# Youngju-Na/UFORecon

Measured on AMD Instinct MI355X. Metric: rays/s (per-ray volume-rendering path, 64+64 hierarchical samples, DTU-shaped 3-view 512x640), higher is better.
Workload: dtype f32; 1 GPU; configs[1]: full 512x640 frame = 327680 rays, 3 source views, 64+64 samples, rays sharded by row tiles over 1 GPU(s), depth/RGB tiles all-gathered; rays_per_frame=327680, chunk_rays=4096, side_streams=3

## Files before the change

### uforecon_amd/csrc/api_ray.hip

```cpp
#include "api_common.h"

using namespace ufr;
using namespace ufr::api;

namespace {
__global__ void order_pe_kernel(float* __restrict__ table, int SN) {
  int i = blockIdx.x * blockDim.x + threadIdx.x;
  if (i >= SN * 8) return;
  int pos = i >> 3, jj = i & 7;
  double ang = (double)pos / pow(10000.0, 2.0 * (double)(jj / 2) / 8.0);
  table[i] = (float)((jj & 1) ? cos(ang) : sin(ang));
}
}

namespace ufr {
hipError_t launch_order_pe(float* table, int SN, hipStream_t s) {
  hipLaunchKernelGGL(order_pe_kernel, dim3((SN * 8 + 255) / 256), dim3(256), 0, s, table, SN);
  return hipGetLastError();
}
}

namespace {
struct AggregateWs { float *token0, *order_pe; };
AggregateWs carve_aggregate(Carver& c, int RN, int SN) {
  AggregateWs w;
  w.token0 = c.f32((size_t)RN * SN * UFR_TOKEN_DIM);
  w.order_pe = c.f32((size_t)SN * 8);
  return w;
}

int aggregate_impl(const void* packed, const float* x_tokens, const float* x_point, const float* rgb, const float* dir, int RN, int SN,
                   int NV, float* radiance, float* srdf, float* token0, float* order_pe, bool pe_ready,
                   float* view_out, float* ray_out, bool lowp, int* status, hipStream_t s) {
  UFR_REQUIRE((unsigned long long)RN * SN * (NV + 1) * UFR_TOKEN_DIM < (1ull << 30),
              "view transformer: %d x %d points x %d tokens exceed the 2^30 token values one call addresses; chunk the points", RN, SN, NV + 1);
  UFR_TIMED("view_transformer", s, launch_view_transformer(static_cast<const float*>(packed), x_tokens, x_point, rgb, dir, RN * SN, NV,
      token0, radiance, view_out, lowp, status, s));
  if (!pe_ready) UFR_HIP(launch_order_pe(order_pe, SN, s));
  UFR_TIMED("ray_transformer", s, launch_ray_transformer(static_cast<const float*>(packed), token0, nullptr, order_pe, RN, SN, srdf,
      ray_out, lowp, status, s));
  return UFR_OK;
}
}

extern "C" {

int ufr_sample_fixed(const float* near, const float* far, const float* U, float* z_out, int32_t RN, int32_t SN,
                     ufr_stream stream) {
  UFR_REQUIRE(near && far && U && z_out, "ufr_sample_fixed: null argument");
  UFR_REQUIRE(RN > 0 && SN >= 2, "ufr_sample_fixed: RN=%d SN=%d", RN, SN);
  UFR_HIP(launch_sample_fixed(near, far, U, RN, z_out, RN, SN, static_cast<hipStream_t>(stream)));
  return UFR_OK;
// ... 23 lines not shown
  return UFR_OK;
}

int ufr_project_gather(const ufr_frame* frame, const ufr_raw_weights* raw, const float* ray_o, int32_t ray_o_stride,
                       const float* ray_d, const float* z, int32_t RN, int32_t SN, float* x_tokens, float* rgb,
                       float* dir, float* sim8, float* vol24, float* xy, float* mask_z, const float* vol24_in,
                       const float* sim8_in, ufr_stream stream) {
  const FrameDev* f = frame_of(frame);
  UFR_REQUIRE(f, "ufr_project_gather: frame handle not prepared");
  UFR_REQUIRE(raw && ray_o && ray_d && z && x_tokens && rgb && dir, "ufr_project_gather: null argument");
  UFR_REQUIRE(ray_o_stride == 0 || ray_o_stride == 3, "ufr_project_gather: ray_o_stride must be 0 or 3");
  UFR_REQUIRE(RN > 0 && SN > 0, "ufr_project_gather: RN=%d SN=%d", RN, SN);
  UFR_REQUIRE(f->match || sim8_in, "ufr_project_gather: the frame has no matching features: sim8_in is required");
  UFR_REQUIRE(f->vol[0] || vol24_in, "ufr_project_gather: the frame has no volumes: vol24_in is required");
  UFR_TIMED("gather", static_cast<hipStream_t>(stream), launch_gather(*f, presim_of(raw), ray_o, ray_o_stride, ray_d, z, RN, SN, x_tokens,
      nullptr, rgb, dir, sim8, vol24, xy, mask_z, vol24_in, sim8_in, static_cast<hipStream_t>(stream)));
  return UFR_OK;
}

size_t ufr_aggregate_workspace_bytes(int32_t RN, int32_t SN, int32_t ) {
  return carved_bytes(carve_aggregate, RN, SN);
}

int ufr_aggregate(const void* packed_weights, const float* x_tokens, const float* rgb, const float* dir, int32_t RN,
                  int32_t SN, int32_t NV, float* radiance, float* srdf, void* workspace, float* view_out,
                  float* ray_out, int32_t precision, ufr_stream stream) {
  UFR_REQUIRE(packed_weights && x_tokens && rgb && dir && radiance && srdf && workspace, "ufr_aggregate: null argument");
  UFR_CHECK(check_views("ufr_aggregate", NV));
  UFR_CHECK(check_ray_samples("ufr_aggregate", RN, SN));
  UFR_PRECISION(precision, lowp, "ufr_aggregate");
  hipStream_t s = static_cast<hipStream_t>(stream);
  UFR_STATUS_ENTER(sl, s, "ufr_aggregate");
  Carver c(workspace);
  const AggregateWs w = carve_aggregate(c, RN, SN);
  UFR_CHECK(aggregate_impl(packed_weights, x_tokens, nullptr, rgb, dir, RN, SN, NV, radiance, srdf, w.token0, w.order_pe, false,
                           view_out, ray_out, lowp, status_word(sl), s));
  return status_leave(sl, s);
}

int ufr_composite(const float* z, const float* radiance, const int32_t* row, const float* srdf, const float* variance,
                  int32_t RN, int32_t SN, float* rgb, float* depth, float* opacity, float* weight, ufr_stream stream) {
  UFR_REQUIRE(z && radiance && srdf && variance && depth, "ufr_composite: null argument");
  UFR_REQUIRE(RN > 0 && SN >= 2 && SN <= 256, "ufr_composite: SN=%d out of range [2,256]", SN);
  UFR_TIMED("composite", static_cast<hipStream_t>(stream), launch_composite(z, radiance, row, srdf, variance, RN, SN, rgb, depth, opacity,
      weight, nullptr, nullptr, static_cast<hipStream_t>(stream)));
  return UFR_OK;
}

int ufr_view_transform(const void* packed_weights, const float* x_tokens, const float* rgb, const float* dir, int32_t P,
                       int32_t NV, float* token0, float* radiance, int32_t precision, ufr_stream stream) {
  UFR_REQUIRE(packed_weights && x_tokens && rgb && dir && token0 && radiance, "ufr_view_transform: null argument");
  UFR_CHECK(check_views("ufr_view_transform", NV));
  UFR_REQUIRE(P > 0, "ufr_view_transform: P=%d", P);
  UFR_PRECISION(precision, lowp, "ufr_view_transform");
  hipStream_t s = static_cast<hipStream_t>(stream);
  UFR_STATUS_ENTER(sl, s, "ufr_view_transform");
  UFR_REQUIRE((unsigned long long)P * (NV + 1) * UFR_TOKEN_DIM < (1ull << 30),
              "ufr_view_transform: %d points x %d tokens exceed the 2^30 token values one call addresses; chunk the points", P, NV + 1);
  UFR_TIMED("view_transformer", s, launch_view_transformer(static_cast<const float*>(packed_weights), x_tokens, nullptr, rgb, dir, P, NV,
      token0, radiance, nullptr, lowp, status_word(sl), s));
  return status_leave(sl, s);
}

size_t ufr_ray_transform_workspace_bytes(int32_t SN) { return align_up((size_t)(SN > 0 ? SN : 1) * 8 * sizeof(float)); }

int ufr_ray_transform(const void* packed_weights, const float* token0, const int32_t* row, int32_t RN, int32_t SN,
                      float* srdf, void* workspace, int32_t precision, ufr_stream stream) {
  UFR_REQUIRE(packed_weights && token0 && srdf && workspace, "ufr_ray_transform: null argument");
  UFR_CHECK(check_ray_samples("ufr_ray_transform", RN, SN));
  UFR_PRECISION(precision, lowp, "ufr_ray_transform");
  hipStream_t s = static_cast<hipStream_t>(stream);
  UFR_STATUS_ENTER(sl, s, "ufr_ray_transform");
  float* order_pe = static_cast<float*>(workspace);
  UFR_HIP(launch_order_pe(order_pe, SN, s));
  UFR_TIMED("ray_transformer", s, launch_ray_transformer(static_cast<const float*>(packed_weights), token0, row, order_pe, RN, SN, srdf,
      nullptr, lowp, status_word(sl), s));
  return status_leave(sl, s);
}

int32_t ufr_default_chunk_rays(void) { return 4096; }

}

namespace {
struct RenderWs {
  float *ray_o, *rd, *near, *far, *camz, *z1, *w1, *srdf1, *depth1, *rgb1, *z2, *srdf2, *rad, *x, *xp, *rgbm, *dir, *token0,
      *pe1, *pe2, *z_new;
  int* row;
  size_t bytes;
};
RenderWs carve_render(void* ws, int R, int SN, int PN, int NV) {
  const size_t S2 = (size_t)SN + PN, Smax = S2 > (size_t)SN ? S2 : SN, Sg = (size_t)(SN > PN ? SN : PN);
  Carver c(ws);
  RenderWs r;
  r.ray_o = c.f32(4);
  r.rd = c.f32((size_t)R * 3);
  r.near = c.f32(R);
  r.far = c.f32(R);
  r.camz = c.f32(R);
  r.z1 = c.f32((size_t)R * SN);
  r.w1 = c.f32((size_t)R * SN);
  r.srdf1 = c.f32((size_t)R * SN);
  r.depth1 = c.f32(R);
  r.rgb1 = c.f32((size_t)R * 3);
  r.z2 = c.f32((size_t)R * S2);
  r.srdf2 = c.f32((size_t)R * S2);
  r.rad = c.f32((size_t)R * Smax * 3);
  r.x = c.f32((size_t)R * Sg * NV * kViewCols);
  r.xp = c.f32((size_t)R * Sg * kPointCols);
  r.rgbm = c.f32((size_t)R * Sg * NV * 4);
  r.dir = c.f32((size_t)R * Sg * NV * 4);
  r.z_new = c.f32((size_t)R * (PN > 0 ? PN : 1));
  r.row = c.take<int>((size_t)R * S2);
  r.token0 = c.f32((size_t)R * Smax * UFR_TOKEN_DIM);
  r.pe1 = c.f32((size_t)SN * 8);
  r.pe2 = c.f32(S2 * 8);
  r.bytes = c.off;
  return r;
}

constexpr int kMaxLanes = 4;
struct SidePool {
  hipStream_t s[kMaxLanes] = {};
  hipEvent_t fork = nullptr, join[kMaxLanes] = {};
  int n = 0;
};
// ... 19 lines not shown
                 int* status, hipStream_t s) {
  const int RN = a->RN, SN = a->SN, PN = a->coarse_only ? 0 : a->PN, NV = f->NV;
  const PreSim ps = presim_of(a->raw);
  const int S2 = SN + PN, HW = f->H * f->W;
  {
    ProfScope p("sampler", s);
    UFR_HIP(launch_ray_setup(a->ray_idx + r0, a->ray_d, a->cam_ray_d, HW, a->near_z, a->far_z, R, w.rd, w.near, w.far,
                             w.camz, a->ray_o, w.ray_o, s));
    UFR_HIP(launch_sample_fixed(w.near, w.far, a->U1 + r0, RN, w.z1, R, SN, s));
    if (!pe_ready) {
      UFR_HIP(launch_order_pe(w.pe1, SN, s));
      if (!a->coarse_only) UFR_HIP(launch_order_pe(w.pe2, S2, s));
      pe_ready = true;
    }
  }
  UFR_TIMED("gather", s, launch_gather(*f, ps, w.ray_o, 0, w.rd, w.z1, R, SN, w.x, w.xp, w.rgbm, w.dir, nullptr, nullptr, nullptr,
      nullptr, nullptr, nullptr, s));
  UFR_CHECK(aggregate_impl(a->packed_weights, w.x, w.xp, w.rgbm, w.dir, R, SN, NV, w.rad, w.srdf1, w.token0, w.pe1, true,
                           nullptr, nullptr, lowp, status, s));
  const bool last = a->coarse_only != 0;
  UFR_TIMED("composite", s, launch_composite(w.z1, w.rad, nullptr, w.srdf1, a->raw->variance, R, SN,
      last ? a->rgb + 3 * (size_t)r0 : w.rgb1, last ? a->depth + r0 : w.depth1, nullptr, w.w1, w.camz,
      (last && a->depth_z) ? a->depth_z + r0 : nullptr, s));
  if (last) {
    if (a->srdf) UFR_HIP(hipMemcpyAsync(a->srdf + (size_t)r0 * SN, w.srdf1, (size_t)R * SN * 4, hipMemcpyDeviceToDevice, s));
    if (a->z_all) UFR_HIP(hipMemcpyAsync(a->z_all + (size_t)r0 * SN, w.z1, (size_t)R * SN * 4, hipMemcpyDeviceToDevice, s));
    return UFR_OK;
  }
  UFR_TIMED("sampler", s, launch_importance_merge(w.w1, w.z1, a->U2 + r0, RN, nullptr, w.z2, R, SN, PN, w.z_new, w.row, s));
  UFR_TIMED("gather", s, launch_gather(*f, ps, w.ray_o, 0, w.rd, w.z_new, R, PN, w.x, w.xp, w.rgbm, w.dir, nullptr, nullptr, nullptr,
      nullptr, nullptr, nullptr, s));
  UFR_TIMED("view_transformer", s, launch_view_transformer(static_cast<const float*>(a->packed_weights), w.x, w.xp, w.rgbm, w.dir, R * PN,
      NV, w.token0 + (size_t)R * SN * UFR_TOKEN_DIM, w.rad + (size_t)R * SN * 3, nullptr, lowp, status, s));
  UFR_TIMED("ray_transformer", s, launch_ray_transformer(static_cast<const float*>(a->packed_weights), w.token0, w.row, w.pe2, R, S2,
      w.srdf2, nullptr, lowp, status, s));
  UFR_TIMED("composite", s, launch_composite(w.z2, w.rad, w.row, w.srdf2, a->raw->variance, R, S2, a->rgb + 3 * (size_t)r0, a->depth + r0,
      nullptr, nullptr, w.camz, a->depth_z ? a->depth_z + r0 : nullptr, s));
  if (a->srdf) UFR_HIP(hipMemcpyAsync(a->srdf + (size_t)r0 * S2, w.srdf2, (size_t)R * S2 * 4, hipMemcpyDeviceToDevice, s));
  if (a->z_all) UFR_HIP(hipMemcpyAsync(a->z_all + (size_t)r0 * S2, w.z2, (size_t)R * S2 * 4, hipMemcpyDeviceToDevice, s));
  return UFR_OK;
}
}

extern "C" {

size_t ufr_render_workspace_bytes(int32_t chunk_rays, int32_t SN, int32_t PN, int32_t NV) {
  if (chunk_rays <= 0) chunk_rays = ufr_default_chunk_rays();
// ... 69 lines not shown
```

### uforecon_amd/csrc/gather.hip

```cpp
#include <algorithm>
#include <cstdlib>
#include "ufr_device.h"
#include "ufr_internal.h"
#include "volume_sample.h"

namespace ufr {

__device__ __forceinline__ f32x4 lerp_tap4_buf(__amdgpu_buffer_rsrc_t r, unsigned base, int stride_bytes, const Tap2& t, unsigned c4) {
  f32x4 v[4];
#pragma unroll
  for (int k = 0; k < 4; ++k)
    v[k] = buf_ld4(r, t.o[k] >= 0 ? base + __umul24((unsigned)t.o[k], (unsigned)stride_bytes) + c4 : kBufOut);
  f32x4 acc;
#pragma unroll
  for (int e = 0; e < 4; ++e) {
    float a = mul_rn(v[0][e], t.w[0]);
    a = fmaf(v[1][e], t.w[1], a);
    a = fmaf(v[2][e], t.w[2], a);
    acc[e] = fmaf(v[3][e], t.w[3], a);
  }
  return acc;
}

typedef int i32x4 __attribute__((ext_vector_type(4)));
// ... 88 lines not shown
#define UFR_G_PHASE(i)                                                                 \
  {                                                                                    \
    const unsigned long long t_now = __builtin_readcyclecounter();                     \
    g_acc[i] = t_now - g_prev;                                                         \
    g_prev = t_now;                                                                    \
  }
#else
#define UFR_G_PHASE(i)
#endif

template <int NVT>
__global__ void __launch_bounds__(64 * NVT, kGatherMinW) gather_kernel(FrameDev f, PreSim ps, const float* __restrict__ ray_o,
                                                      int o_stride, const float* __restrict__ ray_d,
                                                      const float* __restrict__ zval, int P, int SN, int SG,
                                                      float* __restrict__ x_tokens, float* __restrict__ x_point,
                                                      float* __restrict__ rgb_out,
                                                      float* __restrict__ dir_out, float* __restrict__ sim8_out,
                                                      float* __restrict__ vol24_out, float* __restrict__ xy_out,
                                                      float* __restrict__ maskz_out,
                                                      const float* __restrict__ vol24_in,
                                                      const float* __restrict__ sim8_in) {
  extern __shared__ __attribute__((aligned(16))) float smem[];
  constexpr int NV = NVT;
  constexpr int npair = NV * (NV - 1) / 2;
  float* sh_sim = smem;
  float* sh_tapF = sh_sim + 64 * npair * 8;
  float* sh_tapM = sh_tapF + NV * 64 * 8;
  float* sh_vol = sh_tapF;
  constexpr int sim_slot = npair * 8;
  constexpr bool out_in_sim = sim_slot >= 48;
  float* sh_out = out_in_sim ? sh_sim + 8 : sh_tapF;
// ... 1 lines not shown
#ifdef UFR_PHASE_TIMING
  unsigned long long g_acc[8] = {};
  unsigned long long g_prev = __builtin_readcyclecounter();
#endif

  const int v = threadIdx.x >> 6, p = threadIdx.x & 63;
  const int vu = __builtin_amdgcn_readfirstlane(v);
  const int nb8 = (int)(gridDim.x / 8) * 8;
  const int blk = (int)blockIdx.x < nb8 ? (int)(blockIdx.x % 8) * (nb8 / 8) + (int)(blockIdx.x / 8) : (int)blockIdx.x;
  int pbase = blk * 64;
  if (SG) {
    const int rg = blk / SG;
    pbase = (kBlkRays * rg) * SN + kBlkSamples * (blk - rg * SG);
  }
  const auto point_of = [=](int lp) { return SG ? pbase + (int)((unsigned)lp % kBlkRays) * SN + (int)((unsigned)lp / kBlkRays) : pbase + lp; };
  const int pidx = point_of(p);
  const bool active = pidx < P;
  const int pc = active ? pidx : P - 1;
  const int ray = pc / SN;

  const float zz = zval[pc];
  const float* o = ray_o + (size_t)ray * o_stride;
  const float px = mul_add_unfused(zz, ray_d[3 * ray + 0], o[0]);
  const float py = mul_add_unfused(zz, ray_d[3 * ray + 1], o[1]);
  const float pz = mul_add_unfused(zz, ray_d[3 * ray + 2], o[2]);

  const float* M = f.pose[v];
  float qx = fmaf(M[2], pz, fmaf(M[1], py, mul_rn(M[0], px))) + M[3];
  float qy = fmaf(M[6], pz, fmaf(M[5], py, mul_rn(M[4], px))) + M[7];
  float qz = fmaf(M[10], pz, fmaf(M[9], py, mul_rn(M[8], px))) + M[11];
  const float mask_z = qz > 0.f ? 1.f : 0.f;
  const float x = qx / qz, y = qy / qz;
  if (active && xy_out) {
    xy_out[((size_t)v * P + pidx) * 2 + 0] = x;
    xy_out[((size_t)v * P + pidx) * 2 + 1] = y;
  }
  if (active && maskz_out) maskz_out[(size_t)v * P + pidx] = mask_z;

  const int row_cols = x_point ? kViewCols : UFR_TOKEN_DIM, pe_col = x_point ? 32 : 72;
  float* xrow = x_tokens + ((size_t)pc * NV + v) * row_cols;

  {
    put_tap(sh_tapF + (v * 64 + p) * 8, taps_zeros(unnorm2d_nac(x, f.w), unnorm2d_nac(y, f.h), f.w, f.h));
    put_tap(sh_tapM + (v * 64 + p) * 8, taps_border(unnorm2d_ac(x, f.w), unnorm2d_ac(y, f.h), f.w, f.h));
    Tap2 tf = taps_zeros(unnorm2d_nac(x, f.W), unnorm2d_nac(y, f.H), f.W, f.H);
    const unsigned img_px = (unsigned)(f.H * f.W);
    f32x4 c4 = lerp_tap4_buf(buf_rsrc(f.rgb + (size_t)vu * img_px * 4, img_px * 16u), 0u, 16, tf, 0u);
    const float inb = (x <= 1.f && x >= -1.f && y <= 1.f && y >= -1.f) ? 1.f : 0.f;
    c4[3] = inb * mask_z;
    if (active) st4(rgb_out + ((size_t)pidx * NV + v) * 4, c4);
    float dv[4];
    const __amdgpu_buffer_rsrc_t rdepth = buf_rsrc(f.depth + (size_t)vu * img_px, img_px * 4u);
#pragma unroll
    for (int k = 0; k < 4; ++k) dv[k] = buf_ld1(rdepth, tf.o[k] >= 0 ? (unsigned)tf.o[k] * 4u : kBufOut);
    const float dm = fmaf(dv[3], tf.w[3], fmaf(dv[2], tf.w[2], fmaf(dv[1], tf.w[1], mul_rn(dv[0], tf.w[0]))));
    const float* R = f.w2c_z[v];
    float zc = fmaf(R[2], pz, fmaf(R[1], py, mul_rn(R[0], px))) + R[3];
    float delta = dm - zc;
    float pe[8];
#pragma unroll
    for (int k = 0; k < 4; ++k) {
      const float fr = 3.14159274101257324f * (float)(1 << k);
      pe[2 * k] = sinf(mul_rn(delta, fr));
      pe[2 * k + 1] = sinf(fmaf(delta, fr, 1.57079637050628662f));
    }
    if (active) {
      st4(xrow + pe_col, f32x4{pe[0], pe[1], pe[2], pe[3]});
      st4(xrow + pe_col + 4, f32x4{pe[4], pe[5], pe[6], pe[7]});
    }
    float ax = px - f.ref_pos[0], ay = py - f.ref_pos[1], az = pz - f.ref_pos[2];
    float bx = px - f.cam_pos[v][0], by = py - f.cam_pos[v][1], bz = pz - f.cam_pos[v][2];
    const float ra = __builtin_amdgcn_rcpf(sqrtf(ax * ax + ay * ay + az * az));
    const float rb = __builtin_amdgcn_rcpf(sqrtf(bx * bx + by * by + bz * bz));
    if (active) st4(dir_out + ((size_t)pidx * NV + v) * 4, f32x4{ax * ra - bx * rb, ay * ra - by * rb, az * ra - bz * rb, 0.f});
  }

  __syncthreads();
  UFR_G_PHASE(0)

  const int c8 = threadIdx.x & 7, grp = threadIdx.x >> 3;
  constexpr int n_grp = 64 * NV / 8;
  const unsigned map_px = (unsigned)(f.h * f.w);
  const __amdgpu_buffer_rsrc_t rfeat = buf_rsrc(f.feat, (unsigned)NV * map_px * 128u);
  const __amdgpu_buffer_rsrc_t rmatch = buf_rsrc(f.match, (unsigned)NV * map_px * (unsigned)f.match_ch * 4u);
  for (int item = grp; item < 64 * NV; item += n_grp) {
    const int iv = item >> 6, ip = item & 63;
    const int ipidx = point_of(ip);
    if (ipidx < P) {
      const Tap2 t = get_tap(sh_tapF + (iv * 64 + ip) * 8);
// ... 9 lines not shown
    const int b = a + rem;
    const int va = a, ca = b, vb = b + 1, cb = a;
    const Tap2 ta = get_tap(sh_tapM + (va * 64 + ip) * 8), tb = get_tap(sh_tapM + (vb * 64 + ip) * 8);
    const unsigned mrow = (unsigned)f.match_ch * 4u;
    f32x4 fa = lerp_tap4_buf(rmatch, (unsigned)va * map_px * mrow + 128u * ca, (int)mrow, ta, 16u * c8);
    f32x4 fb = lerp_tap4_buf(rmatch, (unsigned)vb * map_px * mrow + 128u * cb, (int)mrow, tb, 16u * c8);
    float na = fmaxf(sqrtf(fa[0] * fa[0] + fa[1] * fa[1] + fa[2] * fa[2] + fa[3] * fa[3]), 1e-8f);
    float nb = fmaxf(sqrtf(fb[0] * fb[0] + fb[1] * fb[1] + fb[2] * fb[2] + fb[3] * fb[3]), 1e-8f);
    const float ra = __builtin_amdgcn_rcpf(na), rb = __builtin_amdgcn_rcpf(nb);
    sh_sim[(ip * npair + q) * 8 + c8] = (fa[0] * ra) * (fb[0] * rb) + (fa[1] * ra) * (fb[1] * rb) +
                                        (fa[2] * ra) * (fb[2] * rb) + (fa[3] * ra) * (fb[3] * rb);
  }
  __syncthreads();
  UFR_G_PHASE(1)

  float own[25];
  if (vol24_in) {
#pragma unroll
    for (int c = 0; c < 25; ++c) own[c] = 0.f;
  } else {
    const float zn = ((qz - f.vol_near) / (f.vol_far - f.vol_near)) * 2.f - 1.f;
    float fl[24], wl = 0.f;
#pragma unroll
    for (int s = 0; s < UFR_NUM_STAGES; ++s) {
      float fs[8], ws;
      const float* vol = f.vol[s];
      const unsigned vox = (unsigned)(f.vD[s] * f.vH[s] * f.vW[s]);
      sample_volume_buf(buf_rsrc(vol + (size_t)vu * vox * kVolCh, vox * (unsigned)(kVolCh * 4)), f.vD[s], f.vH[s], f.vW[s], x, y, zn,
                        fs, ws);
#pragma unroll
      for (int c = 0; c < 8; ++c) fl[8 * s + c] = fs[c];
      wl = s == 0 ? ws : wl + ws;
    }
#pragma unroll
    for (int c = 0; c < 24; ++c) own[c] = fl[c] * wl;
    own[24] = wl;
    if (v > 0) {
      float* dst = sh_vol + (p * (NV - 1) + (v - 1)) * 25;
#pragma unroll
      for (int c = 0; c < 25; ++c) dst[c] = own[c];
    }
  }
  __syncthreads();
  UFR_G_PHASE(2)

  if (v == 0) {
    float sim[8];
#pragma unroll
    for (int gi = 0; gi < 8; ++gi) {
      float s = 0.f;
      for (int q = 0; q < npair; ++q) s += sh_sim[(p * npair + q) * 8 + gi];
      sim[gi] = s / (float)npair;
      if (sim8_in) sim[gi] = sim8_in[(size_t)pc * 8 + gi];
    }
    {
      float Wsum = own[24];
// ... 13 lines not shown
    float* mine = sh_sim + p * sim_slot;
    st4(mine, f32x4{sim[0], sim[1], sim[2], sim[3]});
    st4(mine + 4, f32x4{sim[4], sim[5], sim[6], sim[7]});
    float* ov = sh_out + p * out_stride;
#pragma unroll
    for (int c = 0; c < 24; c += 4) st4(ov + c, f32x4{own[c], own[c + 1], own[c + 2], own[c + 3]});
    UFR_G_PHASE(3)
    __builtin_amdgcn_fence(__ATOMIC_RELEASE, "wavefront");
    __builtin_amdgcn_wave_barrier();
    __builtin_amdgcn_fence(__ATOMIC_ACQUIRE, "wavefront");
    presim_block(ps, sh_sim, sim_slot, sh_out, out_stride, p);
  }
  __syncthreads();
  UFR_G_PHASE(4)

  int npts = P - pbase < 64 ? P - pbase : 64;
  if (SG) {
    const int nrays = (P - pbase + SN - 1) / SN;
    npts = nrays < kBlkRays ? kBlkSamples * nrays : 64;
  }
  const auto local_of = [=](int j) { return SG ? (int)((unsigned)j % kBlkSamples) * kBlkRays + (int)((unsigned)j / kBlkSamples) : j; };
  if (x_point) {
    for (int i = threadIdx.x; i < npts * 10; i += 64 * NV) {
      const int j = i / 10, c = i - j * 10, ip = local_of(j);
      st4(x_point + (size_t)point_of(ip) * kPointCols + 4 * c, ld4(sh_out + ip * out_stride + 4 * c));
    }
  } else {
    for (int i = threadIdx.x; i < npts * NV * 10; i += 64 * NV) {
      const int row = i / 10, c = i - row * 10, j = row / NV, ip = local_of(j);
      st4(x_tokens + ((size_t)point_of(ip) * NV + (row - j * NV)) * UFR_TOKEN_DIM + 32 + 4 * c, ld4(sh_out + ip * out_stride + 4 * c));
    }
  }
  if (vol24_out)
    for (int i = threadIdx.x; i < npts * 24; i += 64 * NV) {
      const int j = i / 24, ip = local_of(j);
      vol24_out[(size_t)point_of(ip) * 24 + (i - j * 24)] = sh_out[ip * out_stride + (i - j * 24)];
// ... 1 lines not shown
  if (sim8_out)
    for (int i = threadIdx.x; i < npts * 8; i += 64 * NV) {
      const int ip = local_of(i >> 3);
      sim8_out[(size_t)point_of(ip) * 8 + (i & 7)] = sh_sim[ip * sim_slot + (i & 7)];
    }
  UFR_G_PHASE(5)
#ifdef UFR_PHASE_TIMING
  if (threadIdx.x == 0) {
    for (int i = 0; i < 6; ++i) atomicAdd(&g_gather_phase[i], g_acc[i]);
    atomicAdd(&g_gather_phase[6], 1ull);
  }
#endif
}

hipError_t launch_gather(const FrameDev& f, const PreSim& ps, const float* ray_o, int o_stride, const float* ray_d,
                         const float* z, int RN, int SN, float* x_tokens, float* x_point, float* rgb, float* dir, float* sim8,
                         float* vol24, float* xy, float* mask_z, const float* vol24_in, const float* sim8_in,
                         hipStream_t s) {
  const int P = RN * SN, NV = f.NV;
  const int npair = NV * (NV - 1) / 2;
  const size_t taps = 2 * (size_t)NV * 64 * 8, volp = (size_t)64 * (NV - 1) * 25, outv = npair * 8 >= 48 ? 0 : 64 * 40;
  size_t lds = sizeof(float) * ((size_t)64 * npair * 8 + std::max(std::max(taps, volp), outv));
  const int SG = (SN % kBlkSamples == 0 && RN >= kBlkRays) ? SN / kBlkSamples : 0;
  const int blocks = SG ? ((RN + kBlkRays - 1) / kBlkRays) * SG : (P + 63) / 64;
  switch (NV) {
#define UFR_GATHER_CASE(N)                                                                                                   \
    case N:                                                                                                                  \
      hipLaunchKernelGGL(gather_kernel<N>, dim3(blocks), dim3(64 * N), lds, s, f, ps, ray_o, o_stride, ray_d, z, P, SN, SG, \
                         x_tokens, x_point, rgb, dir, sim8, vol24, xy, mask_z, vol24_in, sim8_in);                          \
      break;
    UFR_GATHER_CASE(2) UFR_GATHER_CASE(3) UFR_GATHER_CASE(4) UFR_GATHER_CASE(5) UFR_GATHER_CASE(6) UFR_GATHER_CASE(7)
#undef UFR_GATHER_CASE
    default: return hipErrorInvalidValue;
  }
  return hipGetLastError();
}

}

#ifdef UFR_PHASE_TIMING
extern "C" int ufr_debug_gather_phases(unsigned long long* out, int n, int reset) {
  unsigned long long h[32] = {};
  if (hipMemcpyFromSymbol(h, HIP_SYMBOL(ufr::g_gather_phase), sizeof(h)) != hipSuccess) return -1;
  for (int i = 0; i < n && i < 32; ++i) out[i] = h[i];
// ... 8 lines not shown
```

### uforecon_amd/csrc/ufr_internal.h

```cpp
#pragma once
#include <hip/hip_runtime.h>
#include <stdint.h>

#include <mutex>

#include "../../include/ufr.h"
#include "ufr_layout.h"

namespace ufr {

constexpr int kVolCh = 12;

struct FrameDev {
  int32_t NV, H, W, h, w, match_ch;
  const float* feat;
  const float* match;
  const float* rgb;
  const float* depth;
  const float* vol[UFR_NUM_STAGES];
  int32_t vD[UFR_NUM_STAGES], vH[UFR_NUM_STAGES], vW[UFR_NUM_STAGES];
  float pose[UFR_MAX_VIEWS][12];
  float cam_pos[UFR_MAX_VIEWS][3];
  float w2c_z[UFR_MAX_VIEWS][4];
  float ref_pos[3];
// ... 19 lines not shown
  }
};

hipError_t launch_nchw_to_nhwc(const float* in, float* out, int N, int C, int S, int Cpad, hipStream_t s, unsigned* abs_max = nullptr);
hipError_t launch_volume_pack(const float* feat, const float* weight, float* out, int N, int S, hipStream_t s, unsigned* abs_max = nullptr);
hipError_t launch_ray_setup(const int64_t* ray_idx, const float* ray_d, const float* cam_ray_d, int HW, float near_z,
                            float far_z, int RN, float* rd_out, float* near_out, float* far_out, float* camz_out,
                            const float* ray_o_host, float* ray_o_out, hipStream_t s);
hipError_t launch_sample_fixed(const float* near, const float* far, const float* U, int u_stride, float* z, int RN,
                               int SN, hipStream_t s);
hipError_t launch_importance_merge(const float* weight, const float* z, const float* U2, int u_stride, float* z_fine,
                                   float* z_all, int RN, int SN, int PN, float* z_new, int* src_row, hipStream_t s);
hipError_t launch_order_pe(float* table, int SN, hipStream_t s);
hipError_t launch_points(const float* ray_o, int o_stride, const float* ray_d, const float* z, float* pts, int RN,
                         int SN, hipStream_t s);
constexpr int kViewCols = 40, kPointCols = 40;
hipError_t launch_gather(const FrameDev& f, const PreSim& ps, const float* ray_o, int o_stride, const float* ray_d,
                         const float* z, int RN, int SN, float* x_tokens, float* x_point, float* rgb, float* dir, float* sim8,
                         float* vol24, float* xy, float* mask_z, const float* vol24_in, const float* sim8_in,
                         hipStream_t s);
hipError_t launch_view_transformer(const float* packed, const float* x_tokens, const float* x_point, const float* rgb,
                                   const float* dir, int P, int NV, float* token0, float* radiance, float* view_out, bool lowp, int* status,
                                   hipStream_t s);
hipError_t launch_ray_transformer(const float* packed, const float* token0, const int* tok_row, const float* order_pe,
                                  int RN, int SN, float* srdf, float* ray_out, bool lowp, int* status, hipStream_t s);
hipError_t launch_composite(const float* z, const float* radiance, const int* rad_row, const float* srdf,
                            const float* variance, int RN, int SN, float* rgb, float* depth, float* opacity, float* weight,
                            const float* camz, float* depth_z, hipStream_t s);
hipError_t launch_render_loss(const float* rgb_c, const float* depth_c, const float* rgb_f, const float* depth_f,
                              const float* rgb_gt, const float* depth_gt, const float* near_far, int nf_stride, int B, int RN,
                              float weight_rgb, float weight_depth, float* loss, float* d_rgb_c, float* d_depth_c,
                              float* d_rgb_f, float* d_depth_f, hipStream_t s);
hipError_t launch_composite_bwd(const float* z, const float* radiance, const int* rad_row, bool accumulate, const float* srdf,
                                const float* variance, int RN, int SN, const float* d_rgb, const float* d_depth,
                                const float* d_opacity, const float* d_weight, float* d_radiance, float* d_srdf,
                                float* d_variance, hipStream_t s);
struct GradPtrs;
int view_tape_blocks(int P, int NV);
// ... 121 lines not shown
```

### uforecon_amd/csrc/view_transformer.hip

```cpp
#include <cstdlib>
#include "bwd_tape.h"
#include "ufr_internal.h"
#include "weight_stream_f16.h"

namespace ufr {

template <class T>
__device__ __forceinline__ T* at32(T* base, unsigned elem) {
  typedef typename std::conditional<std::is_const<T>::value, const char, char>::type B;
  return reinterpret_cast<T*>(reinterpret_cast<B*>(base) + (elem * (unsigned)sizeof(T)));
}

template <int C, int N>
__device__ __forceinline__ void zero_tiles(f32x4 (&t)[C][N]) {
#pragma unroll
  for (int c = 0; c < C; ++c)
#pragma unroll
    for (int i = 0; i < N; ++i) t[c][i] = splat4(0.f);
}

template <int C, int VW, int VB, class WS>
__device__ __forceinline__ void layer_norm80(f32x4 (&t)[C][5], const WS& ws, int g, float eps, float asc, f32x4 (*XH)[5] = nullptr, float* RS = nullptr) {
#pragma unroll
  for (int c = 0; c < C; ++c) {
// ... 121 lines not shown
  for (int it = 0; it < n_iter; ++it) {
    const int grp = it * n_waves + wave_global;
    const bool wrap = it + 1 < n_iter;
    typedef ViewTapeLayout<LOWP> TapeL;
    const int col0 = __builtin_amdgcn_readfirstlane(grp < n_groups ? grp : 0) * C;
    char* const tape_blk = reinterpret_cast<char*>(tape) + (size_t)(col0 / kBlockCols) * (TapeL::block_units * 512);
    auto tape_st = [&](int tile, int c, f32x4 v) __attribute__((always_inline)) {
      if (grp < n_groups) tile_store<TapeL>(tape_blk, tile, col0 % kBlockCols + c, lane, v);
    };
    f32x4 x[C][5];
    int pidx[C];
    bool valid[C];
    auto load_x = [&](int c, f32x4 (&dst)[5]) __attribute__((always_inline)) {
      const int pp = valid[c] ? pidx[c] : 0;
      const int tv = tvv[c];
      const unsigned vrow = ((unsigned)pp * NV + (tv > 0 ? tv - 1 : 0)) * (x_point ? kViewCols : UFR_TOKEN_DIM);
      const unsigned prow_e = x_point ? (unsigned)pp * kPointCols : vrow + 32;
      const float* pbase = x_point ? x_point : x_tokens;
      const float* row = at32(x_tokens, vrow + 4 * g);
      const float* prow = at32(pbase, prow_e + 4 * g);
      const float* last = g < 2 ? prow + 32 : row + (x_point ? 32 : 72) - 8;
#pragma unroll
      for (int t = 0; t < 5; ++t) {
        f32x4 tok = vec_frag<V_VIEW_TOKEN>(ws, t, g);
        f32x4 val = ld4(t < 2 ? row + 16 * t : t < 4 ? prow + 16 * (t - 2) : last);
        dst[t] = tv == 0 ? tok : val;
        if (!valid[c]) dst[t] = splat4(0.f);
      }
    };
#pragma unroll
    for (int c = 0; c < C; ++c) {
      pidx[c] = grp * PPW + ptw[c];
      valid[c] = okc[c] && grp < n_groups && pidx[c] < P;
      load_x(c, x[c]);
    }
    track_external(x, ws);
// ... 258 lines not shown
#pragma unroll
          for (int r = 0; r < 4; ++r)
            if (hid[c][t][r] > 0.f) relu_bits[c][(4 * t + r) >> 5] |= 1u << ((4 * t + r) & 31);
        }
    }
    zero_tiles(o);
    gemm_f16<M_VT_MLP2, C, kVtWaves>(ws, hid, o, wrap, sc[VS_M_MLP2]);
    f32x4 col[C];
    float dcomp[C];
#pragma unroll
    for (int c = 0; c < C; ++c) {
      col[c] = splat4(0.f);
      dcomp[c] = 0.f;
      const int tv = tvv[c];
      if (valid[c] && tv > 0) {
        col[c] = ld4(at32(rgbm, ((unsigned)pidx[c] * NV + (tv - 1)) * 4u));
        dcomp[c] = *at32(dirs, ((unsigned)pidx[c] * NV + (tv - 1)) * 4u + g);
      }
    }

    UFR_PHASE(8)
    if constexpr (TAPE) {
      f32x4 xh[C][5];
      layer_norm80<C, V_VT_N2W, V_VT_N2B>(o, ws, g, sc[VS_EPS2], sc[VS_MLP2_ASC], xh, rstd2);
#pragma unroll
      for (int c = 0; c < C; ++c)
#pragma unroll
        for (int t = 0; t < 5; ++t) tape_st(TV_XH2 + t, c, xh[c][t]);
    } else {
      layer_norm80<C, V_VT_N2W, V_VT_N2B>(o, ws, g, sc[VS_EPS2], 1.f);
    }
#pragma unroll
// ... 148 lines not shown
    g_vt_phase[21] += __builtin_readcyclecounter() - t_start;
  }
  if (lane == 0 && wave_global < 4096) {
    unsigned xcc;
    asm volatile("s_getreg_b32 %0, hwreg(HW_REG_XCC_ID)" : "=s"(xcc));
    unsigned hwid;
    asm volatile("s_getreg_b32 %0, hwreg(HW_REG_HW_ID)" : "=s"(hwid));
    g_vt_wave[2 * wave_global] = t_start;
    g_vt_wave[2 * wave_global + 1] = (__builtin_readcyclecounter() - t_start) | ((unsigned long long)(xcc & 0xf) << 60) |
                                     ((unsigned long long)(hwid & 0xffff) << 40);
  }
#endif
}

template <int L, bool LOWP, bool TAPE = false>
static hipError_t launch_vt(const float* packed, const float* x_tokens, const float* x_point, const float* rgb, const float* dir, int P,
                            float* token0, float* radiance, float* view_out, int* status, hipStream_t s, float* tape = nullptr) {
  constexpr int C = TAPE ? 1 : kVtC;
  constexpr int PPW = (L == 6 && C == 2 && !TAPE) ? 5 : (16 / L) * C;
  const int n_groups = TAPE ? ((P + (16 / L) * kBlockCols - 1) / ((16 / L) * kBlockCols)) * (kBlockCols / C) : (P + PPW - 1) / PPW;
  int blocks = (n_groups + kVtWaves - 1) / kVtWaves;
  constexpr int resident = 256 * (kVtMinW * 4 / kVtWaves);
  const int max_blocks = resident * kVtOversub;
  if (blocks > max_blocks) {
    const int base = (n_groups + max_blocks * kVtWaves - 1) / (max_blocks * kVtWaves);
    long best_cost = -1;
    for (int n_iter = base; n_iter <= 4 * base; ++n_iter) {
      const int b = (n_groups + kVtWaves * n_iter - 1) / (kVtWaves * n_iter);
      const long cost = (long)((b + resident - 1) / resident) * n_iter;
      if (best_cost < 0 || cost < best_cost) { best_cost = cost; blocks = b; }
    }
  }
// ... 2 lines not shown
  hipLaunchKernelGGL((view_transformer_kernel<L, C, LOWP, TAPE>), dim3(blocks), dim3(kVtBlock), kF16LdsBytes, s, packed, x_tokens,
                     x_point, rgb, dir, P, token0, radiance, view_out, status, tape);
  return hipGetLastError();
}

int view_tape_blocks(int P, int NV) {
  const int PPW = (16 / (NV + 1)) * kBlockCols;
  return (P + PPW - 1) / PPW;
}
hipError_t launch_view_tape(const float* packed, const float* x_tokens, const float* rgb, const float* dir, int P, int NV,
                            float* token0, float* radiance, float* tape, bool lowp, int* status, hipStream_t s) {
  if (P <= 0 || (unsigned long long)P * (NV + 1) * UFR_TOKEN_DIM >= (1ull << 30)) return hipErrorInvalidValue;
  switch (NV) {
#define UFR_VT_CASE(N)                                                                                                   \
    case N:                                                                                                              \
      return lowp ? launch_vt<N + 1, true, true>(packed, x_tokens, nullptr, rgb, dir, P, token0, radiance, nullptr, status, s, tape) \
                  : launch_vt<N + 1, false, true>(packed, x_tokens, nullptr, rgb, dir, P, token0, radiance, nullptr, status, s, tape);
    UFR_VT_CASE(2) UFR_VT_CASE(3) UFR_VT_CASE(4) UFR_VT_CASE(5) UFR_VT_CASE(6) UFR_VT_CASE(7)
#undef UFR_VT_CASE
    default: return hipErrorInvalidValue;
  }
}

hipError_t launch_view_transformer(const float* packed, const float* x_tokens, const float* x_point, const float* rgb,
                                   const float* dir, int P, int NV, float* token0, float* radiance, float* view_out, bool lowp, int* status,
                                   hipStream_t s) {
  if (P <= 0 || (unsigned long long)P * (NV + 1) * UFR_TOKEN_DIM >= (1ull << 30)) return hipErrorInvalidValue;
  switch (NV) {
#define UFR_VT_CASE(N)                                                                                       \
    case N:                                                                                                  \
      return lowp ? launch_vt<N + 1, true>(packed, x_tokens, x_point, rgb, dir, P, token0, radiance, view_out, status, s)     \
                  : launch_vt<N + 1, false>(packed, x_tokens, x_point, rgb, dir, P, token0, radiance, view_out, status, s);
    UFR_VT_CASE(2) UFR_VT_CASE(3) UFR_VT_CASE(4) UFR_VT_CASE(5) UFR_VT_CASE(6) UFR_VT_CASE(7)
#undef UFR_VT_CASE
    default: return hipErrorInvalidValue;
  }
}

}

#ifdef UFR_PHASE_TIMING
extern "C" int ufr_debug_vt_phases(unsigned long long* out, int n, int reset) {
  unsigned long long h[32] = {};
  if (hipMemcpyFromSymbol(h, HIP_SYMBOL(ufr::g_vt_phase), sizeof(h)) != hipSuccess) return -1;
  for (int i = 0; i < n && i < 32; ++i) out[i] = h[i];
  if (reset) {
    unsigned long long z[32] = {};
// ... 9 lines not shown
```

Measured before the change: 2.756 million rays/s.

## Pack per-view PE, RGB and direction into a compact small-row buffer

The render path's gather kernel used to write three separate buffers: 40-wide view rows holding positional encodings, an RGB+mask buffer and a direction buffer. It now writes a 32-column feature row plus a 16-float per-view 'small' row (PE, RGB, dir) staged through LDS and stored cooperatively in coalesced form. The view transformer reads PE, RGB and dir from that packed row using shifted offsets. The goal is fewer, better-coalesced global stores and loads. The cost is an extra LDS round trip and extra barriers in the gather kernel.

```diff
diff --git a/uforecon_amd/csrc/api_ray.hip b/uforecon_amd/csrc/api_ray.hip
--- a/uforecon_amd/csrc/api_ray.hip
+++ b/uforecon_amd/csrc/api_ray.hip
@@ -29,13 +29,13 @@
   return w;
 }
 
-int aggregate_impl(const void* packed, const float* x_tokens, const float* x_point, const float* rgb, const float* dir, int RN, int SN,
-                   int NV, float* radiance, float* srdf, float* token0, float* order_pe, bool pe_ready,
+int aggregate_impl(const void* packed, const float* x_tokens, const float* x_point, const float* x_small, const float* rgb,
+                   const float* dir, int RN, int SN, int NV, float* radiance, float* srdf, float* token0, float* order_pe, bool pe_ready,
                    float* view_out, float* ray_out, bool lowp, int* status, hipStream_t s) {
   UFR_REQUIRE((unsigned long long)RN * SN * (NV + 1) * UFR_TOKEN_DIM < (1ull << 30),
               "view transformer: %d x %d points x %d tokens exceed the 2^30 token values one call addresses; chunk the points", RN, SN, NV + 1);
-  UFR_TIMED("view_transformer", s, launch_view_transformer(static_cast<const float*>(packed), x_tokens, x_point, rgb, dir, RN * SN, NV,
-      token0, radiance, view_out, lowp, status, s));
+  UFR_TIMED("view_transformer", s, launch_view_transformer(static_cast<const float*>(packed), x_tokens, x_point, x_small, rgb, dir,
+      RN * SN, NV, token0, radiance, view_out, lowp, status, s));
   if (!pe_ready) UFR_HIP(launch_order_pe(order_pe, SN, s));
   UFR_TIMED("ray_transformer", s, launch_ray_transformer(static_cast<const float*>(packed), token0, nullptr, order_pe, RN, SN, srdf,
       ray_out, lowp, status, s));
@@ -89,7 +89,7 @@
   UFR_REQUIRE(f->match || sim8_in, "ufr_project_gather: the frame has no matching features: sim8_in is required");
   UFR_REQUIRE(f->vol[0] || vol24_in, "ufr_project_gather: the frame has no volumes: vol24_in is required");
   UFR_TIMED("gather", static_cast<hipStream_t>(stream), launch_gather(*f, presim_of(raw), ray_o, ray_o_stride, ray_d, z, RN, SN, x_tokens,
-      nullptr, rgb, dir, sim8, vol24, xy, mask_z, vol24_in, sim8_in, static_cast<hipStream_t>(stream)));
+      nullptr, nullptr, rgb, dir, sim8, vol24, xy, mask_z, vol24_in, sim8_in, static_cast<hipStream_t>(stream)));
   return UFR_OK;
 }
 
@@ -108,7 +108,7 @@
   UFR_STATUS_ENTER(sl, s, "ufr_aggregate");
   Carver c(workspace);
   const AggregateWs w = carve_aggregate(c, RN, SN);
-  UFR_CHECK(aggregate_impl(packed_weights, x_tokens, nullptr, rgb, dir, RN, SN, NV, radiance, srdf, w.token0, w.order_pe, false,
+  UFR_CHECK(aggregate_impl(packed_weights, x_tokens, nullptr, nullptr, rgb, dir, RN, SN, NV, radiance, srdf, w.token0, w.order_pe, false,
                            view_out, ray_out, lowp, status_word(sl), s));
   return status_leave(sl, s);
 }
@@ -132,7 +132,7 @@
   UFR_STATUS_ENTER(sl, s, "ufr_view_transform");
   UFR_REQUIRE((unsigned long long)P * (NV + 1) * UFR_TOKEN_DIM < (1ull << 30),
               "ufr_view_transform: %d points x %d tokens exceed the 2^30 token values one call addresses; chunk the points", P, NV + 1);
-  UFR_TIMED("view_transformer", s, launch_view_transformer(static_cast<const float*>(packed_weights), x_tokens, nullptr, rgb, dir, P, NV,
+  UFR_TIMED("view_transformer", s, launch_view_transformer(static_cast<const float*>(packed_weights), x_tokens, nullptr, nullptr, rgb, dir, P, NV,
       token0, radiance, nullptr, lowp, status_word(sl), s));
   return status_leave(sl, s);
 }
@@ -159,7 +159,7 @@
 
 namespace {
 struct RenderWs {
-  float *ray_o, *rd, *near, *far, *camz, *z1, *w1, *srdf1, *depth1, *rgb1, *z2, *srdf2, *rad, *x, *xp, *rgbm, *dir, *token0,
+  float *ray_o, *rd, *near, *far, *camz, *z1, *w1, *srdf1, *depth1, *rgb1, *z2, *srdf2, *rad, *x, *xp, *xs, *token0,
       *pe1, *pe2, *z_new;
   int* row;
   size_t bytes;
@@ -181,10 +181,9 @@
   r.z2 = c.f32((size_t)R * S2);
   r.srdf2 = c.f32((size_t)R * S2);
   r.rad = c.f32((size_t)R * Smax * 3);
-  r.x = c.f32((size_t)R * Sg * NV * kViewCols);
+  r.x = c.f32((size_t)R * Sg * NV * kFeatCols);
+  r.xs = c.f32((size_t)R * Sg * NV * kSmallCols);
   r.xp = c.f32((size_t)R * Sg * kPointCols);
-  r.rgbm = c.f32((size_t)R * Sg * NV * 4);
-  r.dir = c.f32((size_t)R * Sg * NV * 4);
   r.z_new = c.f32((size_t)R * (PN > 0 ? PN : 1));
   r.row = c.take<int>((size_t)R * S2);
   r.token0 = c.f32((size_t)R * Smax * UFR_TOKEN_DIM);
@@ -234,9 +233,9 @@
       pe_ready = true;
     }
   }
-  UFR_TIMED("gather", s, launch_gather(*f, ps, w.ray_o, 0, w.rd, w.z1, R, SN, w.x, w.xp, w.rgbm, w.dir, nullptr, nullptr, nullptr,
-      nullptr, nullptr, nullptr, s));
-  UFR_CHECK(aggregate_impl(a->packed_weights, w.x, w.xp, w.rgbm, w.dir, R, SN, NV, w.rad, w.srdf1, w.token0, w.pe1, true,
+  UFR_TIMED("gather", s, launch_gather(*f, ps, w.ray_o, 0, w.rd, w.z1, R, SN, w.x, w.xp, w.xs, nullptr, nullptr, nullptr, nullptr,
+      nullptr, nullptr, nullptr, nullptr, s));
+  UFR_CHECK(aggregate_impl(a->packed_weights, w.x, w.xp, w.xs, nullptr, nullptr, R, SN, NV, w.rad, w.srdf1, w.token0, w.pe1, true,
                            nullptr, nullptr, lowp, status, s));
   const bool last = a->coarse_only != 0;
   UFR_TIMED("composite", s, launch_composite(w.z1, w.rad, nullptr, w.srdf1, a->raw->variance, R, SN,
@@ -248,9 +247,9 @@
     return UFR_OK;
   }
   UFR_TIMED("sampler", s, launch_importance_merge(w.w1, w.z1, a->U2 + r0, RN, nullptr, w.z2, R, SN, PN, w.z_new, w.row, s));
-  UFR_TIMED("gather", s, launch_gather(*f, ps, w.ray_o, 0, w.rd, w.z_new, R, PN, w.x, w.xp, w.rgbm, w.dir, nullptr, nullptr, nullptr,
-      nullptr, nullptr, nullptr, s));
-  UFR_TIMED("view_transformer", s, launch_view_transformer(static_cast<const float*>(a->packed_weights), w.x, w.xp, w.rgbm, w.dir, R * PN,
+  UFR_TIMED("gather", s, launch_gather(*f, ps, w.ray_o, 0, w.rd, w.z_new, R, PN, w.x, w.xp, w.xs, nullptr, nullptr, nullptr, nullptr,
+      nullptr, nullptr, nullptr, nullptr, s));
+  UFR_TIMED("view_transformer", s, launch_view_transformer(static_cast<const float*>(a->packed_weights), w.x, w.xp, w.xs, nullptr, nullptr, R * PN,
       NV, w.token0 + (size_t)R * SN * UFR_TOKEN_DIM, w.rad + (size_t)R * SN * 3, nullptr, lowp, status, s));
   UFR_TIMED("ray_transformer", s, launch_ray_transformer(static_cast<const float*>(a->packed_weights), w.token0, w.row, w.pe2, R, S2,
       w.srdf2, nullptr, lowp, status, s));
diff --git a/uforecon_amd/csrc/gather.hip b/uforecon_amd/csrc/gather.hip
--- a/uforecon_amd/csrc/gather.hip
+++ b/uforecon_amd/csrc/gather.hip
@@ -126,7 +126,7 @@
                                                       int o_stride, const float* __restrict__ ray_d,
                                                       const float* __restrict__ zval, int P, int SN, int SG,
                                                       float* __restrict__ x_tokens, float* __restrict__ x_point,
-                                                      float* __restrict__ rgb_out,
+                                                      float* __restrict__ x_small, float* __restrict__ rgb_out,
                                                       float* __restrict__ dir_out, float* __restrict__ sim8_out,
                                                       float* __restrict__ vol24_out, float* __restrict__ xy_out,
                                                       float* __restrict__ maskz_out,
@@ -158,6 +158,12 @@
     pbase = (kBlkRays * rg) * SN + kBlkSamples * (blk - rg * SG);
   }
   const auto point_of = [=](int lp) { return SG ? pbase + (int)((unsigned)lp % kBlkRays) * SN + (int)((unsigned)lp / kBlkRays) : pbase + lp; };
+  int npts = P - pbase < 64 ? P - pbase : 64;
+  if (SG) {
+    const int nrays = (P - pbase + SN - 1) / SN;
+    npts = nrays < kBlkRays ? kBlkSamples * nrays : 64;
+  }
+  const auto local_of = [=](int j) { return SG ? (int)((unsigned)j % kBlkSamples) * kBlkRays + (int)((unsigned)j / kBlkSamples) : j; };
   const int pidx = point_of(p);
   const bool active = pidx < P;
   const int pc = active ? pidx : P - 1;
@@ -181,8 +187,9 @@
   }
   if (active && maskz_out) maskz_out[(size_t)v * P + pidx] = mask_z;
 
-  const int row_cols = x_point ? kViewCols : UFR_TOKEN_DIM, pe_col = x_point ? 32 : 72;
-  float* xrow = x_tokens + ((size_t)pc * NV + v) * row_cols;
+  const bool compact = x_point != nullptr;
+  const int row_cols = compact ? kFeatCols : UFR_TOKEN_DIM;
+  f32x4 small[4];
 
   {
     put_tap(sh_tapF + (v * 64 + p) * 8, taps_zeros(unnorm2d_nac(x, f.w), unnorm2d_nac(y, f.h), f.w, f.h));
@@ -192,7 +199,8 @@
     f32x4 c4 = lerp_tap4_buf(buf_rsrc(f.rgb + (size_t)vu * img_px * 4, img_px * 16u), 0u, 16, tf, 0u);
     const float inb = (x <= 1.f && x >= -1.f && y <= 1.f && y >= -1.f) ? 1.f : 0.f;
     c4[3] = inb * mask_z;
-    if (active) st4(rgb_out + ((size_t)pidx * NV + v) * 4, c4);
+    small[2] = c4;
+    if (active && !compact) st4(rgb_out + ((size_t)pidx * NV + v) * 4, c4);
     float dv[4];
     const __amdgpu_buffer_rsrc_t rdepth = buf_rsrc(f.depth + (size_t)vu * img_px, img_px * 4u);
 #pragma unroll
@@ -208,15 +216,19 @@
       pe[2 * k] = sinf(mul_rn(delta, fr));
       pe[2 * k + 1] = sinf(fmaf(delta, fr, 1.57079637050628662f));
     }
-    if (active) {
-      st4(xrow + pe_col, f32x4{pe[0], pe[1], pe[2], pe[3]});
-      st4(xrow + pe_col + 4, f32x4{pe[4], pe[5], pe[6], pe[7]});
+    small[0] = f32x4{pe[0], pe[1], pe[2], pe[3]};
+    small[1] = f32x4{pe[4], pe[5], pe[6], pe[7]};
+    if (active && !compact) {
+      float* xpe = x_tokens + ((size_t)pidx * NV + v) * UFR_TOKEN_DIM + 72;
+      st4(xpe, small[0]);
+      st4(xpe + 4, small[1]);
     }
     float ax = px - f.ref_pos[0], ay = py - f.ref_pos[1], az = pz - f.ref_pos[2];
     float bx = px - f.cam_pos[v][0], by = py - f.cam_pos[v][1], bz = pz - f.cam_pos[v][2];
     const float ra = __builtin_amdgcn_rcpf(sqrtf(ax * ax + ay * ay + az * az));
     const float rb = __builtin_amdgcn_rcpf(sqrtf(bx * bx + by * by + bz * bz));
-    if (active) st4(dir_out + ((size_t)pidx * NV + v) * 4, f32x4{ax * ra - bx * rb, ay * ra - by * rb, az * ra - bz * rb, 0.f});
+    small[3] = f32x4{ax * ra - bx * rb, ay * ra - by * rb, az * ra - bz * rb, 0.f};
+    if (active && !compact) st4(dir_out + ((size_t)pidx * NV + v) * 4, small[3]);
   }
 
   __syncthreads();
@@ -256,6 +268,18 @@
   __syncthreads();
   UFR_G_PHASE(1)
 
+  if (compact) {
+    float* mine = sh_tapF + (p * NV + v) * kSmallCols;
+#pragma unroll
+    for (int c = 0; c < 4; ++c) st4(mine + 4 * c, small[c]);
+    __syncthreads();
+    constexpr int pt_chunks = NV * kSmallCols / 4;
+    for (int i = threadIdx.x; i < npts * pt_chunks; i += 64 * NV) {
+      const int j = i / pt_chunks, c = i - j * pt_chunks, ip = local_of(j);
+      st4(x_small + (size_t)point_of(ip) * (NV * kSmallCols) + 4 * c, ld4(sh_tapF + ip * (NV * kSmallCols) + 4 * c));
+    }
+  }
+
   float own[25];
   if (vol24_in) {
 #pragma unroll
@@ -277,11 +301,12 @@
 #pragma unroll
     for (int c = 0; c < 24; ++c) own[c] = fl[c] * wl;
     own[24] = wl;
-    if (v > 0) {
-      float* dst = sh_vol + (p * (NV - 1) + (v - 1)) * 25;
-#pragma unroll
-      for (int c = 0; c < 25; ++c) dst[c] = own[c];
-    }
+  }
+  if (compact) __syncthreads();
+  if (!vol24_in && v > 0) {
+    float* dst = sh_vol + (p * (NV - 1) + (v - 1)) * 25;
+#pragma unroll
+    for (int c = 0; c < 25; ++c) dst[c] = own[c];
   }
   __syncthreads();
   UFR_G_PHASE(2)
@@ -325,12 +350,6 @@
   __syncthreads();
   UFR_G_PHASE(4)
 
-  int npts = P - pbase < 64 ? P - pbase : 64;
-  if (SG) {
-    const int nrays = (P - pbase + SN - 1) / SN;
-    npts = nrays < kBlkRays ? kBlkSamples * nrays : 64;
-  }
-  const auto local_of = [=](int j) { return SG ? (int)((unsigned)j % kBlkSamples) * kBlkRays + (int)((unsigned)j / kBlkSamples) : j; };
   if (x_point) {
     for (int i = threadIdx.x; i < npts * 10; i += 64 * NV) {
       const int j = i / 10, c = i - j * 10, ip = local_of(j);
@@ -362,9 +381,10 @@
 }
 
 hipError_t launch_gather(const FrameDev& f, const PreSim& ps, const float* ray_o, int o_stride, const float* ray_d,
-                         const float* z, int RN, int SN, float* x_tokens, float* x_point, float* rgb, float* dir, float* sim8,
-                         float* vol24, float* xy, float* mask_z, const float* vol24_in, const float* sim8_in,
+                         const float* z, int RN, int SN, float* x_tokens, float* x_point, float* x_small, float* rgb, float* dir,
+                         float* sim8, float* vol24, float* xy, float* mask_z, const float* vol24_in, const float* sim8_in,
                          hipStream_t s) {
+  if (x_point ? (!x_small || rgb || dir) : (x_small || !rgb || !dir)) return hipErrorInvalidValue;
   const int P = RN * SN, NV = f.NV;
   const int npair = NV * (NV - 1) / 2;
   const size_t taps = 2 * (size_t)NV * 64 * 8, volp = (size_t)64 * (NV - 1) * 25, outv = npair * 8 >= 48 ? 0 : 64 * 40;
@@ -375,7 +395,7 @@
 #define UFR_GATHER_CASE(N)                                                                                                   \
     case N:                                                                                                                  \
       hipLaunchKernelGGL(gather_kernel<N>, dim3(blocks), dim3(64 * N), lds, s, f, ps, ray_o, o_stride, ray_d, z, P, SN, SG, \
-                         x_tokens, x_point, rgb, dir, sim8, vol24, xy, mask_z, vol24_in, sim8_in);                          \
+                         x_tokens, x_point, x_small, rgb, dir, sim8, vol24, xy, mask_z, vol24_in, sim8_in);                 \
       break;
     UFR_GATHER_CASE(2) UFR_GATHER_CASE(3) UFR_GATHER_CASE(4) UFR_GATHER_CASE(5) UFR_GATHER_CASE(6) UFR_GATHER_CASE(7)
 #undef UFR_GATHER_CASE
diff --git a/uforecon_amd/csrc/ufr_internal.h b/uforecon_amd/csrc/ufr_internal.h
--- a/uforecon_amd/csrc/ufr_internal.h
+++ b/uforecon_amd/csrc/ufr_internal.h
@@ -57,14 +57,14 @@
 hipError_t launch_order_pe(float* table, int SN, hipStream_t s);
 hipError_t launch_points(const float* ray_o, int o_stride, const float* ray_d, const float* z, float* pts, int RN,
                          int SN, hipStream_t s);
-constexpr int kViewCols = 40, kPointCols = 40;
+constexpr int kFeatCols = 32, kSmallCols = 16, kPointCols = 40;
 hipError_t launch_gather(const FrameDev& f, const PreSim& ps, const float* ray_o, int o_stride, const float* ray_d,
-                         const float* z, int RN, int SN, float* x_tokens, float* x_point, float* rgb, float* dir, float* sim8,
-                         float* vol24, float* xy, float* mask_z, const float* vol24_in, const float* sim8_in,
+                         const float* z, int RN, int SN, float* x_tokens, float* x_point, float* x_small, float* rgb, float* dir,
+                         float* sim8, float* vol24, float* xy, float* mask_z, const float* vol24_in, const float* sim8_in,
                          hipStream_t s);
-hipError_t launch_view_transformer(const float* packed, const float* x_tokens, const float* x_point, const float* rgb,
-                                   const float* dir, int P, int NV, float* token0, float* radiance, float* view_out, bool lowp, int* status,
-                                   hipStream_t s);
+hipError_t launch_view_transformer(const float* packed, const float* x_tokens, const float* x_point, const float* x_small,
+                                   const float* rgb, const float* dir, int P, int NV, float* token0, float* radiance,
+                                   float* view_out, bool lowp, int* status, hipStream_t s);
 hipError_t launch_ray_transformer(const float* packed, const float* token0, const int* tok_row, const float* order_pe,
                                   int RN, int SN, float* srdf, float* ray_out, bool lowp, int* status, hipStream_t s);
 hipError_t launch_composite(const float* z, const float* radiance, const int* rad_row, const float* srdf,
diff --git a/uforecon_amd/csrc/view_transformer.hip b/uforecon_amd/csrc/view_transformer.hip
--- a/uforecon_amd/csrc/view_transformer.hip
+++ b/uforecon_amd/csrc/view_transformer.hip
@@ -159,12 +159,16 @@
     auto load_x = [&](int c, f32x4 (&dst)[5]) __attribute__((always_inline)) {
       const int pp = valid[c] ? pidx[c] : 0;
       const int tv = tvv[c];
-      const unsigned vrow = ((unsigned)pp * NV + (tv > 0 ? tv - 1 : 0)) * (x_point ? kViewCols : UFR_TOKEN_DIM);
+      const unsigned pv = (unsigned)pp * NV + (tv > 0 ? tv - 1 : 0);
+      const unsigned vrow = pv * (x_point ? kFeatCols : UFR_TOKEN_DIM);
       const unsigned prow_e = x_point ? (unsigned)pp * kPointCols : vrow + 32;
       const float* pbase = x_point ? x_point : x_tokens;
       const float* row = at32(x_tokens, vrow + 4 * g);
       const float* prow = at32(pbase, prow_e + 4 * g);
-      const float* last = g < 2 ? prow + 32 : row + (x_point ? 32 : 72) - 8;
+      const float* pe_base = x_point ? rgbm - 8 : x_tokens + 72;
+      static_assert(kFeatCols == 2 * kSmallCols, "the small row's offset is half the feature row's");
+      const unsigned pe_e = vrow >> (x_point ? 1 : 0);
+      const float* last = g < 2 ? prow + 32 : at32(pe_base, pe_e + 4 * g) - 8;
 #pragma unroll
       for (int t = 0; t < 5; ++t) {
         f32x4 tok = vec_frag<V_VIEW_TOKEN>(ws, t, g);
@@ -453,8 +457,9 @@
       dcomp[c] = 0.f;
       const int tv = tvv[c];
       if (valid[c] && tv > 0) {
-        col[c] = ld4(at32(rgbm, ((unsigned)pidx[c] * NV + (tv - 1)) * 4u));
-        dcomp[c] = *at32(dirs, ((unsigned)pidx[c] * NV + (tv - 1)) * 4u + g);
+        const unsigned cd = ((unsigned)pidx[c] * NV + (tv - 1)) << (x_point ? 6 : 4);
+        col[c] = ld4(reinterpret_cast<const float*>(reinterpret_cast<const char*>(rgbm) + cd));
+        dcomp[c] = *reinterpret_cast<const float*>(reinterpret_cast<const char*>(dirs) + (cd + 4u * g));
       }
     }
 
@@ -633,8 +638,11 @@
 }
 
 template <int L, bool LOWP, bool TAPE = false>
-static hipError_t launch_vt(const float* packed, const float* x_tokens, const float* x_point, const float* rgb, const float* dir, int P,
-                            float* token0, float* radiance, float* view_out, int* status, hipStream_t s, float* tape = nullptr) {
+static hipError_t launch_vt(const float* packed, const float* x_tokens, const float* x_point, const float* x_small, const float* rgb,
+                            const float* dir, int P, float* token0, float* radiance, float* view_out, int* status, hipStream_t s,
+                            float* tape = nullptr) {
+  if (x_point ? (!x_small || rgb || dir) : (x_small || !rgb || !dir)) return hipErrorInvalidValue;
+  if (x_point) { rgb = x_small + 8; dir = x_small + 12; }
   constexpr int C = TAPE ? 1 : kVtC;
   constexpr int PPW = (L == 6 && C == 2 && !TAPE) ? 5 : (16 / L) * C;
   const int n_groups = TAPE ? ((P + (16 / L) * kBlockCols - 1) / ((16 / L) * kBlockCols)) * (kBlockCols / C) : (P + PPW - 1) / PPW;
@@ -667,23 +675,23 @@
   switch (NV) {
 #define UFR_VT_CASE(N)                                                                                                   \
     case N:                                                                                                              \
-      return lowp ? launch_vt<N + 1, true, true>(packed, x_tokens, nullptr, rgb, dir, P, token0, radiance, nullptr, status, s, tape) \
-                  : launch_vt<N + 1, false, true>(packed, x_tokens, nullptr, rgb, dir, P, token0, radiance, nullptr, status, s, tape);
+      return lowp ? launch_vt<N + 1, true, true>(packed, x_tokens, nullptr, nullptr, rgb, dir, P, token0, radiance, nullptr, status, s, tape) \
+                  : launch_vt<N + 1, false, true>(packed, x_tokens, nullptr, nullptr, rgb, dir, P, token0, radiance, nullptr, status, s, tape);
     UFR_VT_CASE(2) UFR_VT_CASE(3) UFR_VT_CASE(4) UFR_VT_CASE(5) UFR_VT_CASE(6) UFR_VT_CASE(7)
 #undef UFR_VT_CASE
     default: return hipErrorInvalidValue;
   }
 }
 
-hipError_t launch_view_transformer(const float* packed, const float* x_tokens, const float* x_point, const float* rgb,
-                                   const float* dir, int P, int NV, float* token0, float* radiance, float* view_out, bool lowp, int* status,
-                                   hipStream_t s) {
+hipError_t launch_view_transformer(const float* packed, const float* x_tokens, const float* x_point, const float* x_small,
+                                   const float* rgb, const float* dir, int P, int NV, float* token0, float* radiance,
+                                   float* view_out, bool lowp, int* status, hipStream_t s) {
   if (P <= 0 || (unsigned long long)P * (NV + 1) * UFR_TOKEN_DIM >= (1ull << 30)) return hipErrorInvalidValue;
   switch (NV) {
 #define UFR_VT_CASE(N)                                                                                       \
     case N:                                                                                                  \
-      return lowp ? launch_vt<N + 1, true>(packed, x_tokens, x_point, rgb, dir, P, token0, radiance, view_out, status, s)     \
-                  : launch_vt<N + 1, false>(packed, x_tokens, x_point, rgb, dir, P, token0, radiance, view_out, status, s);
+      return lowp ? launch_vt<N + 1, true>(packed, x_tokens, x_point, x_small, rgb, dir, P, token0, radiance, view_out, status, s) \
+                  : launch_vt<N + 1, false>(packed, x_tokens, x_point, x_small, rgb, dir, P, token0, radiance, view_out, status, s);
     UFR_VT_CASE(2) UFR_VT_CASE(3) UFR_VT_CASE(4) UFR_VT_CASE(5) UFR_VT_CASE(6) UFR_VT_CASE(7)
 #undef UFR_VT_CASE
     default: return hipErrorInvalidValue;
```

Result: no change. 2.777 million rays/s (median of 6 runs) (+0.8%).
